# Sbte/RAILS

Hardware: AMD Instinct MI355X
Metric: RAILS iterations/sec (+ A*V SpMM HBM GB/s in roofline), m=1M rows/GPU, k=128, fp64 (higher is better)
Workload: dtype f64

## Files before the change

include/rails_hip.h:

```cpp
#ifndef RAILS_HIP_H
#define RAILS_HIP_H

#include <stddef.h>
#include <stdint.h>

#ifdef __cplusplus
extern "C" {
#endif

#define RAILS_OK 0
#define RAILS_EINVAL -1
#define RAILS_EHIP -2
#define RAILS_ENOMEM -3
#define RAILS_ELAPACK -4
#define RAILS_ECOMM -5
#define RAILS_ENODEV -6

typedef struct rails_ctx rails_ctx;
typedef struct rails_csr rails_csr;
typedef struct rails_panel rails_panel;

const char *rails_last_error(void);
const char *rails_version(void);

// ... 95 lines not shown

int rails_panel_gemm(rails_ctx *ctx, double alpha, const rails_panel *X, int xc0, int k, const double *C_host,
                     int ldc, int r, double beta, rails_panel *Y, int yc0);

int rails_ctx_enable_library_gemm(rails_ctx *ctx);
int rails_ctx_library_gemm_ready(const rails_ctx *ctx);

int rails_deferred_reserve(rails_ctx *ctx, int nslots, int64_t doubles_per_slot);
int rails_gram_deferred(rails_ctx *ctx, const rails_panel *X, int xc0, int a, const rails_panel *Y, int yc0, int b, int slot);
int rails_panel_gemm_deferred(rails_ctx *ctx, double alpha, const rails_panel *X, int xc0, int k, int slot, int ld, int r, double beta,
                              rails_panel *Y, int yc0);
int rails_chol_inverse_deferred(rails_ctx *ctx, int slot_in, int w, int slot_out);
int rails_update_gram_deferred(rails_ctx *ctx, double alpha, const rails_panel *X, int xc0, int k, const double *C_host, int ldc, int r,
                               rails_panel *Y, int yc0, int r2, int slot);
int rails_deferred_fetch(rails_ctx *ctx, int slot, int64_t n, double *host_out);

int rails_panel_gemm_wide(rails_ctx *ctx, double alpha, const rails_panel *X, int xc0, int k, const double *C_host, int ldc, int r,
                          double beta, rails_panel *Y, int yc0);

int rails_orthogonalize(rails_ctx *ctx, rails_panel *V, int k_old, int w, int method, int *used);
int rails_orthogonalize_deflated(rails_ctx *ctx, rails_panel *V, int k_old, int w, const rails_panel *N, int nc0, int q, int method, int *used);

int rails_resid_lanczos(rails_ctx *ctx, const rails_panel *AV, int avc0, const rails_panel *MV, int mvc0, int k,
                        const double *T_host, int ldt, const rails_panel *B, int bc0, int p, int L,
                        double *H_host, int ldh, int *steps);

int rails_lanczos_start(rails_ctx *ctx, const rails_panel *AV, int avc0, const rails_panel *MV, int mvc0, int k,
                        const rails_panel *B, int bc0, int p, double *sums_host);

int rails_lanczos_vectors(rails_ctx *ctx, const double *S_host, int lds, int w, rails_panel *Out, int oc0);
// ... 29 lines not shown
```

rails_amd/_lib.py:

```python
import ctypes as C
import os

_HERE = os.path.dirname(os.path.abspath(__file__))
LIB_PATH = os.path.join(_HERE, "lib", "librails_hip.so")

_dp = C.POINTER(C.c_double)
_ip = C.POINTER(C.c_int)
_i64p = C.POINTER(C.c_int64)
_i32p = C.POINTER(C.c_int32)
_vp = C.c_void_p

ALLREDUCE_FN = C.CFUNCTYPE(C.c_int, C.c_void_p, C.c_void_p, C.c_size_t, C.c_void_p)
HALO_FN = C.CFUNCTYPE(C.c_int, C.c_void_p, C.c_void_p, C.c_void_p, C.c_int, C.c_void_p)
APPLY_FN = C.CFUNCTYPE(C.c_int, C.c_void_p, C.c_int, C.c_void_p, C.c_int, C.c_int, C.c_void_p, C.c_int)

SIGNATURES = {
    "rails_last_error": (C.c_char_p, []),
    "rails_version": (C.c_char_p, []),
    "rails_ctx_create": (C.c_int, [C.c_int, _vp, C.POINTER(_vp)]),
    "rails_ctx_destroy": (C.c_int, [_vp]),
    "rails_ctx_sync": (C.c_int, [_vp]),
    "rails_ctx_stream": (_vp, [_vp]),
    "rails_ctx_set_meter": (C.c_int, [_vp, C.c_int]),
    "rails_ctx_enable_library_gemm": (C.c_int, [_vp]),
    "rails_ctx_library_gemm_ready": (C.c_int, [_vp]),
    "rails_deferred_reserve": (C.c_int, [_vp, C.c_int, C.c_int64]),
    "rails_gram_deferred": (C.c_int, [_vp, _vp, C.c_int, C.c_int, _vp, C.c_int, C.c_int, C.c_int]),
    "rails_update_gram_deferred": (C.c_int, [_vp, C.c_double, _vp, C.c_int, C.c_int, _dp, C.c_int, C.c_int, _vp, C.c_int, C.c_int, C.c_int]),
    "rails_panel_gemm_deferred": (C.c_int, [_vp, C.c_double, _vp, C.c_int, C.c_int, C.c_int, C.c_int, C.c_int, C.c_double, _vp, C.c_int]),
    "rails_chol_inverse_deferred": (C.c_int, [_vp, C.c_int, C.c_int, C.c_int]),
    "rails_deferred_fetch": (C.c_int, [_vp, C.c_int, C.c_int64, _dp]),
    "rails_ctx_stats": (C.c_int, [_vp, C.c_char_p, C.c_int]),
    "rails_ctx_set_seed": (C.c_int, [_vp, C.c_uint64, C.c_uint64]),
    "rails_ctx_rng_state": (C.c_int, [_vp, C.POINTER(C.c_uint64), C.POINTER(C.c_uint64)]),
    "rails_ctx_set_partition": (C.c_int, [_vp, C.c_int, C.c_int, C.c_int64, C.c_int64]),
    "rails_ctx_set_allreduce": (C.c_int, [_vp, ALLREDUCE_FN, _vp]),
    "rails_rccl_unique_id": (C.c_int, [_vp]),
    "rails_ctx_init_rccl": (C.c_int, [_vp, _vp, C.c_int, C.c_int]),
    "rails_ctx_set_rccl": (C.c_int, [_vp, _vp]),
    "rails_ctx_rccl_size": (C.c_int, [_vp]),
    "rails_csr_set_halo_counts": (C.c_int, [_vp, C.c_int, _i64p, _i64p]),
    "rails_csr_create": (C.c_int, [_vp, C.c_int64, C.c_int64, _i64p, _i32p, _dp, C.POINTER(_vp)]),
    "rails_csr_create_rect": (C.c_int, [_vp, C.c_int64, C.c_int64, _i64p, _i32p, _dp, C.POINTER(_vp)]),
    "rails_csr_create_callback": (C.c_int, [_vp, C.c_int64, APPLY_FN, _vp, C.POINTER(_vp)]),
    "rails_csr_destroy": (C.c_int, [_vp]),
    "rails_csr_rows": (C.c_int64, [_vp]),
# ... 103 lines not shown
```

rails_amd/csrc/ctx.hip:

```cpp
#include "rails_internal.h"

static thread_local char g_err[1024] = "";

void rails_set_error(const char *fmt, ...)
{
    va_list ap;
    va_start(ap, fmt);
    vsnprintf(g_err, sizeof(g_err), fmt, ap);
    va_end(ap);
}

extern "C" const char *rails_last_error(void) { return g_err; }
extern "C" const char *rails_version(void) { return "rails_amd 0.1 (gfx950)"; }


extern "C" int rails_ctx_create(int device, void *stream, rails_ctx **out)
{
    RAILS_REQUIRE(out != nullptr, "rails_ctx_create: out is null");
    int ndev = 0;
    hipError_t e = hipGetDeviceCount(&ndev);
    if (e != hipSuccess || ndev <= 0) {
        rails_set_error("rails_ctx_create: no HIP device visible (%s); the HIP path has no CPU fallback",
                        e == hipSuccess ? "device count 0" : hipGetErrorString(e));
        return RAILS_ENODEV;
// ... 39 lines not shown
extern "C" int rails_ctx_destroy(rails_ctx *c)
{
    if (!c) return RAILS_OK;
    hipSetDevice(c->device);
    rails_stream_sync(c);
    rails_lanczos_release(c);
    rails_rccl_release(c);
    rails_library_gemm_release(c);
    for (auto &fp : c->free_panels) hipFree(fp.second);
    c->free_panels.clear();
    if (c->ws) hipFree(c->ws);
    if (c->small) hipFree(c->small);
    if (c->pinned) hipHostFree(c->pinned);
    if (c->defer_dev) hipFree(c->defer_dev);
    if (c->defer_pin) hipHostFree(c->defer_pin);
    if (c->ev0) hipEventDestroy(c->ev0);
    if (c->ev1) hipEventDestroy(c->ev1);
    if (c->ev_h2d) hipEventDestroy(c->ev_h2d);
    for (hipEvent_t e : c->meter_events) hipEventDestroy(e);
    if (c->stream2) hipStreamDestroy(c->stream2);
    if (c->ev_fork) hipEventDestroy(c->ev_fork);
    if (c->ev_join) hipEventDestroy(c->ev_join);
    if (c->own_stream) hipStreamDestroy(c->stream);
    delete c;
    return RAILS_OK;
}

int rails_ctx_second_stream(rails_ctx *c)
{
    if (c->stream2) return RAILS_OK;
// ... 477 lines not shown
```

rails_amd/csrc/dense.hip:

```cpp
#include "rails_internal.h"

#include <dlfcn.h>
#include <atomic>
#include <mutex>

#include <algorithm>

namespace {

typedef double v4f64 __attribute__((ext_vector_type(4)));
typedef double v2f64 __attribute__((ext_vector_type(2)));

__device__ __forceinline__ v4f64 mfma_f64(double a, double b, v4f64 c)
{
    return __builtin_amdgcn_mfma_f64_16x16x4f64(a, b, c, 0, 0, 0);
}

struct OneSeg {
    const double *X;
    int ld;
    struct Row {
        const double *x;
    };
    __device__ int col(int c) const { return c; }
// ... 368 lines not shown
    RAILS_HIP_CHECK(hipMemcpyAsync(c->pinned, c->small, n * sizeof(double), hipMemcpyDeviceToHost, c->stream));
    RAILS_HIP_CHECK(rails_stream_sync(c));
    for (int j = 0; j < b; ++j) memcpy(C_host + (size_t)j * ldc, c->pinned + (size_t)j * a, sizeof(double) * a);
    return RAILS_OK;
}


namespace {

__global__ void k_compact_cols(const double *__restrict__ src, int ld, int k, int r, double *__restrict__ dst)
{
    const int64_t n = (int64_t)k * r;
    for (int64_t q = (int64_t)blockIdx.x * blockDim.x + threadIdx.x; q < n; q += (int64_t)gridDim.x * blockDim.x) dst[q] = src[(q / k) * ld + (q % k)];
}

__global__ __launch_bounds__(64) void k_small_chol(const double *__restrict__ G, int w, double *__restrict__ M)
{
    constexpr int LD = 49;
    __shared__ double S[48 * LD], Ri[48 * LD], d[48];
    const int t = threadIdx.x;
    const bool mine = t < w;
    for (int q = t; q < w * w; q += 64) S[(q / w) * LD + (q % w)] = G[q];
    __syncthreads();
    if (mine) d[t] = sqrt(S[t * LD + t]);
    __syncthreads();
    for (int q = t; q < w * w; q += 64) S[(q / w) * LD + (q % w)] /= d[q % w] * d[q / w];
    __syncthreads();
    for (int i = 0; i < w; ++i) {
        const double piv = sqrt(S[i * LD + i]);
        double rij = 0.0;
        if (mine && t >= i) rij = (t == i) ? piv : S[t * LD + i] / piv;
        __syncthreads();
        if (mine && t >= i) S[t * LD + i] = rij;
        __syncthreads();
        if (mine && t > i)
            for (int l = i + 1; l <= t; ++l) S[t * LD + l] -= S[l * LD + i] * rij;
        __syncthreads();
    }
    if (mine) {
        for (int l = 0; l < w; ++l) Ri[t * LD + l] = 0.0;
        for (int i = t; i >= 0; --i) {
            double s = (i == t) ? 1.0 : 0.0;
            for (int l = i + 1; l <= t; ++l) s -= S[l * LD + i] * Ri[t * LD + l];
            Ri[t * LD + i] = s / S[i * LD + i];
        }
    }
    __syncthreads();
    for (int q = t; q < w * w; q += 64) {
        const int j = q / w, i = q % w;
        M[q] = i <= j ? Ri[j * LD + i] / d[i] : 0.0;
    }
}

}

extern "C" int rails_deferred_reserve(rails_ctx *c, int nslots, int64_t doubles_per_slot)
{
    RAILS_REQUIRE(c && nslots >= 1 && doubles_per_slot >= 1, "rails_deferred_reserve: bad argument");
    hipSetDevice(c->device);
    if (c->defer_dev && c->defer_nslots >= nslots && c->defer_slot >= (size_t)doubles_per_slot) return RAILS_OK;
    RAILS_HIP_CHECK(rails_stream_sync(c));
    if (c->defer_dev) hipFree(c->defer_dev);
    if (c->defer_pin) hipHostFree(c->defer_pin);
    c->defer_dev = c->defer_pin = nullptr;
    const size_t slot = ((size_t)doubles_per_slot * 3 / 2 + 63) / 64 * 64, bytes = slot * (size_t)nslots * sizeof(double);
    c->n_dev_alloc++;
    RAILS_HIP_CHECK(hipMalloc((void **)&c->defer_dev, bytes));
    RAILS_HIP_CHECK(hipHostMalloc((void **)&c->defer_pin, bytes, hipHostMallocDefault));
    c->defer_slot = slot;
    c->defer_nslots = nslots;
    return RAILS_OK;
}

#define RAILS_SLOT_CHECK(slot, n, what)                                                                                                    \
    RAILS_REQUIRE(c && c->defer_dev && (slot) >= 0 && (slot) < c->defer_nslots && (size_t)(n) <= c->defer_slot,                            \
                  what ": slot %d / %lld doubles outside the arena (rails_deferred_reserve)", (int)(slot), (long long)(n))

extern "C" int rails_gram_deferred(rails_ctx *c, const rails_panel *X, int xc0, int a, const rails_panel *Y, int yc0, int b, int slot)
{
    if (c) hipSetDevice(c->device);
    RAILS_REQUIRE(c && X && Y, "rails_gram_deferred: null argument");
    RAILS_REQUIRE(a >= 1 && b >= 1 && xc0 >= 0 && yc0 >= 0 && xc0 + a <= X->cap && yc0 + b <= Y->cap && X->m == Y->m, "rails_gram_deferred: bad windows");
    const size_t n = (size_t)a * b;
// ... 210 lines not shown
}

extern "C" int rails_chol_inverse_deferred(rails_ctx *c, int slot_in, int w, int slot_out)
{
    if (c) hipSetDevice(c->device);
    RAILS_REQUIRE(c && w >= 1 && w <= 48 && slot_in != slot_out, "rails_chol_inverse_deferred: bad argument (w = %d)", w);
    RAILS_SLOT_CHECK(slot_in, (size_t)w * w, "rails_chol_inverse_deferred");
    RAILS_SLOT_CHECK(slot_out, (size_t)w * w, "rails_chol_inverse_deferred");
    RAILS_LAUNCH(k_small_chol, dim3(1), dim3(64), 0, c->stream, c->defer_dev + (size_t)slot_in * c->defer_slot, w, c->defer_dev + (size_t)slot_out * c->defer_slot);
    RAILS_HIP_CHECK(hipGetLastError());
    RAILS_HIP_CHECK(hipMemcpyAsync(c->defer_pin + (size_t)slot_out * c->defer_slot, c->defer_dev + (size_t)slot_out * c->defer_slot, (size_t)w * w * sizeof(double),
                                   hipMemcpyDeviceToHost, c->stream));
    return RAILS_OK;
}

extern "C" int rails_deferred_fetch(rails_ctx *c, int slot, int64_t n, double *host_out)
{
    RAILS_REQUIRE(host_out && n >= 0, "rails_deferred_fetch: bad argument");
    RAILS_SLOT_CHECK(slot, n, "rails_deferred_fetch");
    memcpy(host_out, c->defer_pin + (size_t)slot * c->defer_slot, (size_t)n * sizeof(double));
    return RAILS_OK;
}

int rails_panel_gemm_dev(rails_ctx *c, double alpha, const double *X, int ldx, int k, const double *C_dev, int r, double beta,
                         double *Y, int ldy, int64_t m)
{
    if (r <= 0 || m <= 0) return RAILS_OK;
    int vec_ok = ((((uintptr_t)X) & 15) == 0 && (ldx % 2) == 0) ? 1 : 0;
    int tr = (r + 15) / 16;
    if (tr <= 1)
        launch_pg<1, 32>(c, alpha, X, ldx, k, C_dev, r, beta, Y, ldy, m, vec_ok);
    else if (tr <= 2)
        launch_pg<2, 32>(c, alpha, X, ldx, k, C_dev, r, beta, Y, ldy, m, vec_ok);
    else if (tr <= 4)
// ... 184 lines not shown
```

rails_amd/csrc/dense_panel_gemm.inc:

```
    constexpr int RL = 16 * TR + 4;
    __shared__ double Cs[KC * RL];
    const int lane = threadIdx.x & 63;
    const int wave = threadIdx.x >> 6;
    const int li = lane & 15, kk = lane >> 4;
    const int64_t r0 = ((int64_t)blockIdx.x * 4 + wave) * 16;
    const int64_t myrow = r0 + li;
    const bool rowok = myrow < m;

    v4f64 acc[TR];
#pragma unroll
    for (int t = 0; t < TR; ++t) acc[t] = (v4f64){0.0, 0.0, 0.0, 0.0};

    const auto xrow = Xo.row(myrow);
    for (int kc = 0; kc < k; kc += KC) {
        __syncthreads();
        for (int idx = threadIdx.x; idx < KC * 16 * TR; idx += 256) {
            int kl = idx % KC, j = idx / KC;
            double v = 0.0;
            if (kc + kl < k && j < r) v = C[(kc + kl) + (int64_t)j * k];
            Cs[kl * RL + j] = v;
        }
        __syncthreads();
#pragma unroll
        for (int kb = 0; kb < KC; kb += 16) {
            const int kcol = kc + kb + 4 * kk;
            double xs[4];
            if (rowok && RAILS_PG_VEC4(kcol)) {
                const double *src = Xo.at(xrow, Xo.col(kcol));
                v2f64 t0 = *reinterpret_cast<const v2f64 *>(src);
                v2f64 t1 = *reinterpret_cast<const v2f64 *>(src + 2);
                xs[0] = t0.x;
                xs[1] = t0.y;
                xs[2] = t1.x;
                xs[3] = t1.y;
            } else {
#pragma unroll
                for (int s = 0; s < 4; ++s) xs[s] = (rowok && kcol + s < k) ? *Xo.at(xrow, Xo.col(kcol + s)) : 0.0;
            }
#pragma unroll
            for (int s = 0; s < 4; ++s) {
                const double *crow = &Cs[(kb + 4 * kk + s) * RL + li];
#pragma unroll
                for (int t = 0; t < TR; ++t) acc[t] = mfma_f64(xs[s], crow[16 * t], acc[t]);
            }
        }
    }
#pragma unroll
    for (int t = 0; t < TR; ++t) {
        const int j = 16 * t + li;
        if (j >= r) continue;
#pragma unroll
        for (int v = 0; v < 4; ++v) {
            const int64_t row = r0 + kk + 4 * v;
            if (row >= m) continue;
            double *dst = Yp + row * ldy + j;
            double val = alpha * acc[t][v];
            if (beta != 0.0) val += beta * (*dst);
            *dst = val;
        }
    }
#undef RAILS_PG_VEC4
```

rails_amd/csrc/rails_internal.h:

```cpp
#ifndef RAILS_INTERNAL_H
#define RAILS_INTERNAL_H

#include <hip/hip_runtime.h>

#include <cstdarg>
#include <cstdint>
#include <cstdio>
#include <cstring>
#include <ctime>
#include <string>
#include <vector>

#include "rails_hip.h"

void rails_set_error(const char *fmt, ...);

#define RAILS_HIP_CHECK(expr)                                                                      \
    do {                                                                                           \
        hipError_t e__ = (expr);                                                                   \
        if (e__ != hipSuccess) {                                                                   \
            rails_set_error("%s:%d: %s failed: %s", __FILE__, __LINE__, #expr, hipGetErrorString(e__)); \
            return RAILS_EHIP;                                                                     \
        }                                                                                          \
    } while (0)
// ... 32 lines not shown
    int rccl_nranks = 0, rccl_rank = 0;
    double *ws = nullptr;
    size_t ws_bytes = 0;
    std::vector<std::pair<size_t, double *>> free_panels;
    size_t free_panel_bytes = 0;
    double *small = nullptr;
    size_t small_bytes = 0;
    double *pinned = nullptr;
    size_t pinned_bytes = 0;
    hipEvent_t ev0 = nullptr, ev1 = nullptr;
    hipEvent_t ev_h2d = nullptr;
    bool h2d_pending = false;
    double *defer_dev = nullptr, *defer_pin = nullptr;
    size_t defer_slot = 0;
    int defer_nslots = 0;
    bool meter = false;
    std::vector<hipEvent_t> meter_events;
    int meter_open = 0;
    long meter_missed = 0;
    double gpu_busy_ms = 0.0;
    void *lz = nullptr;
    long n_orth_block = 0, n_orth_columnwise = 0, n_spmm_tiled = 0, n_spmm_planes = 0, n_spmm_overlapped = 0, n_spmm_sweep = 0, n_spmm_rowgather = 0, n_spmm_callback = 0, n_dev_alloc = 0, n_allreduce = 0, n_lanczos = 0, n_lanczos_start = 0, n_orth_repair = 0, n_update_gram_fused = 0, n_rowquad = 0;
};

constexpr int RAILS_METER_PAIRS = 512;
inline bool rails_meter_before(rails_ctx *c)
{
    if (!c->meter) return false;
    if (c->meter_open >= RAILS_METER_PAIRS) {
        c->meter_missed++;
// ... 151 lines not shown
```

rails_amd/csrc/solver_capi.cpp:

```cpp
#include <cmath>
#include <cstdio>
#include <cstring>
#include <map>
#include <string>
#include <vector>

#include <exception>
#include <new>

#include "rails/HipSolverOps.hpp"
#include "rails/SubspaceSolverOps.hpp"
#include "rails_solution.h"
#include "rails_solver.h"

void rails_set_error(const char *fmt, ...);

namespace
{

class ParameterList
{
    std::map<std::string, double> params_;

public:
// ... 226 lines not shown
    rails::SubspaceMultiVector Vc(basis, 1);
    if (s->have_V0) {
        Vc = rails::SubspaceMultiVector::Absorb(basis, s->V);
        Vc.set_orthogonalized(Vc.N());
    }
    int rc = solver.solve(Vc, s->T);
    s->null_rank = solver.nullspace_rank();
    if (rc == -2) return rc;
    s->V = Vc.materialise();
    s->V.set_orthogonalized(s->V.N());
    s->sub_trips = solver.trips();
    s->sub_hist = solver.residual_history();
    s->sub_profile = solver.profile();
    char buf[1536];
    snprintf(buf, sizeof(buf), "{\"dim\": %d, \"absorb\": %ld, \"absorb_columns\": %ld, \"one_by_one\": %ld, \"dropped\": %ld, \"compress\": %ld, \"materialise\": %ld, \"prefetched_random\": %ld, \"second_rounds\": %ld, \"delicate_blocks\": %ld, \"reprojected_blocks\": %ld, \"overlapped_blocks\": %ld, \"replaced_columns\": %ld, \"verified\": %d, \"verify_representation\": %.3e, \"verify_orthonormality\": %.3e, \"seconds\": {\"materialise\": %.4f, \"absorb\": %.4f, \"compress_qr\": %.4f, \"compress_rotate\": %.4f, "
             "\"compress_coefficients\": %.4f}}",
             basis->dim, basis->n_absorb, basis->n_absorb_cols, basis->n_single, basis->n_dropped, basis->n_compress, basis->n_materialise, basis->n_prefetched, basis->n_second_round, basis->n_delicate, basis->n_reprojected, basis->n_overlapped, basis->n_replaced, basis->verify ? 1 : 0, basis->verify_repr, basis->verify_orth,
             basis->t_materialise, basis->t_absorb, basis->t_qr, basis->t_rotate, basis->t_recoef);
    s->sub_stats = buf;
    if (basis->failed) {
        rails_set_error("coordinate-space back end: a device operation failed (%s)", rails_last_error());
        return -1000;
    }
    return rc;
}

extern "C" int rails_solver_solve(rails_solver *s, int *code, int *k)
{
    if (!s) return RAILS_EINVAL;
    const bool restart_from_solution = s->params.get("Restart from solution", 0.0) != 0.0;
    s->last_was_subspace = s->subspace && (s->have_V0 || !restart_from_solution);
    {
        rails::HipSolver::Projection proj;
// ... 149 lines not shown
```

rails_amd/include/rails/SubspaceWrappers.hpp:

```cpp
#ifndef RAILS_SUBSPACEWRAPPERS_HPP
#define RAILS_SUBSPACEWRAPPERS_HPP

#include <algorithm>
#include <atomic>
#include <chrono>
#include <cmath>
#include <cstdlib>
#include <cstring>
#include <iostream>
#include <memory>
#include <vector>

#include "rails/HipWrappers.hpp"

namespace rails
{

struct CoefStore {
    std::vector<double> c;
    int ld = 0, ncap = 0;
    bool in_basis = true;
    CoefStore(int ld_, int ncap_, bool in_basis_) : c((size_t)std::max(ld_, 1) * std::max(ncap_, 1), 0.0), ld(ld_), ncap(std::max(ncap_, 1)), in_basis(in_basis_) {}
    double *col(int j) { return c.data() + (size_t)j * ld; }
    const double *col(int j) const { return c.data() + (size_t)j * ld; }
};

class SubspaceBasis
{
public:
    rails_ctx *ctx;
    int64_t m_local, m_global;
    HipMultiVectorWrapper P, P2;
    int dim = 0;
    int row_cap;
    std::vector<std::weak_ptr<CoefStore>> live;
    long n_absorb = 0, n_absorb_cols = 0, n_single = 0, n_compress = 0, n_materialise = 0, n_dropped = 0, n_prefetched = 0, n_second_round = 0, n_delicate = 0, n_reprojected = 0;
    bool failed = false;
    long n_replaced = 0;
    double t_materialise = 0, t_absorb = 0, t_qr = 0, t_rotate = 0, t_recoef = 0;
    bool profile_sync = getenv("RAILS_SUBSPACE_PROFILE") != nullptr;
    bool trace = getenv("RAILS_SUBSPACE_TRACE") != nullptr;
    double reorth_survival = getenv("RAILS_SUBSPACE_REORTH") ? atof(getenv("RAILS_SUBSPACE_REORTH")) : 0.5;
    double slow_ms = getenv("RAILS_SUBSPACE_SLOW_MS") ? atof(getenv("RAILS_SUBSPACE_SLOW_MS")) : 0.0;
    struct Tick {
        SubspaceBasis *b;
        double *acc;
        const char *what;
        std::chrono::steady_clock::time_point t0;
        Tick(SubspaceBasis *bb, double *a, const char *w = "") : b(bb), acc(a), what(w)
        {
            if (b->profile_sync) rails_ctx_sync(b->ctx);
            t0 = std::chrono::steady_clock::now();
        }
        ~Tick()
        {
            if (b->profile_sync) rails_ctx_sync(b->ctx);
            const double dt = std::chrono::duration<double>(std::chrono::steady_clock::now() - t0).count();
            *acc += dt;
            if (b->slow_ms > 0.0 && dt * 1e3 > b->slow_ms)
                std::cerr << "[subspace] " << what << ": " << dt * 1e3 << " ms (dim " << b->dim << ", absorbs so far " << b->n_absorb << ")" << std::endl;
        }
    };
    std::shared_ptr<CoefStore> cached_random;
    bool cached_valid = false;
    bool prefetch_random = true;

    bool overlap = !(getenv("RAILS_SUBSPACE_OVERLAP") && atoi(getenv("RAILS_SUBSPACE_OVERLAP")) == 0);
    double overlap_min_survival = 1e-4;
    long n_overlapped = 0;
    struct Pending {
        bool active = false;
        int dim0 = 0, w = 0, w2 = 0;
        std::vector<double> Rfp;
        std::vector<double> g0diag;
    } pending;
    enum { SLOT_C2 = 0, SLOT_G = 1, SLOT_M1 = 2, SLOT_G2 = 3, SLOT_M2 = 4, N_SLOTS = 5 };

    SubspaceBasis(rails_ctx *c, int64_t ml, int64_t mg, int rows) : ctx(c), m_local(ml), m_global(mg), P(ml, std::max(rows, 16), c), row_cap(std::max(rows, 16))
    {
        P.set_global_rows(mg);
        P.resize(0);
    }
// ... 375 lines not shown
            d[j] = std::sqrt(Gp[j + (size_t)j * w]);
        }
        std::vector<double> R1((size_t)w * w);
        for (int b = 0; b < w; ++b)
            for (int a = 0; a < w; ++a) R1[a + (size_t)b * w] = Gp[a + (size_t)b * w] / (d[a] * d[b]);
        int info = 0;
        rails_dpotrf('U', w, R1.data(), w, &info);
        if (info != 0) return false;
        for (int a = 0; a < w; ++a)
            if (!(R1[a + (size_t)a * w] > 1e-2)) return false;
        if (!hip_ok(rails_deferred_reserve(ctx, N_SLOTS, (int64_t)(P.capacity() + 64) * (w <= 32 ? 32 : 48)), "rails_deferred_reserve")) return false;
        rails_panel *pp = P.panel();
        bool ok = true;
        if (w2 > 0) {
            ok = ok && hip_ok(rails_update_gram_deferred(ctx, -1.0, pp, 0, dim, CG.data(), dw, w, pp, dim, w2, SLOT_C2), "rails_update_gram_deferred");
            ok = ok && hip_ok(rails_panel_gemm_deferred(ctx, -1.0, pp, 0, dim, SLOT_C2, dim, w2, 1.0, pp, dim), "rails_panel_gemm_deferred");
        } else
            ok = ok && hip_ok(rails_panel_gemm(ctx, -1.0, pp, 0, dim, CG.data(), dw, w, 1.0, pp, dim), "rails_panel_gemm");
        ok = ok && hip_ok(rails_gram_deferred(ctx, pp, dim, w, pp, dim, w, SLOT_G), "rails_gram_deferred");
        ok = ok && hip_ok(rails_chol_inverse_deferred(ctx, SLOT_G, w, SLOT_M1), "rails_chol_inverse_deferred");
        ok = ok && hip_ok(rails_panel_gemm_deferred(ctx, 1.0, pp, dim, w, SLOT_M1, w, w, 0.0, pp, dim), "rails_panel_gemm_deferred");
        ok = ok && hip_ok(rails_gram_deferred(ctx, pp, dim, w, pp, dim, w, SLOT_G2), "rails_gram_deferred");
        ok = ok && hip_ok(rails_chol_inverse_deferred(ctx, SLOT_G2, w, SLOT_M2), "rails_chol_inverse_deferred");
        ok = ok && hip_ok(rails_panel_gemm_deferred(ctx, 1.0, pp, dim, w, SLOT_M2, w, w, 0.0, pp, dim), "rails_panel_gemm_deferred");
        if (!ok) return fail("the overlapped block orthogonalisation could not be queued");
        pending.active = true;
        pending.dim0 = dim;
        pending.w = w;
        pending.w2 = w2;
        pending.Rfp.assign((size_t)w * w, 0.0);
        pending.g0diag.resize(w);
        for (int b = 0; b < w; ++b) {
            pending.g0diag[b] = G0[b + (size_t)b * w];
            for (int a = 0; a <= b; ++a) {
                pending.Rfp[a + (size_t)b * w] = R1[a + (size_t)b * w] * d[b];
                coef[(dim + a) + (size_t)b * ld] = pending.Rfp[a + (size_t)b * w];
            }
        }
        if (w2 > 0) n_second_round++;
// ... 1 lines not shown
        static const long spoil = getenv("RAILS_SUBSPACE_TEST_SPOIL_PREDICTION") ? atol(getenv("RAILS_SUBSPACE_TEST_SPOIL_PREDICTION")) : 0;
        if (spoil > 0 && n_overlapped == spoil) {
            pending.Rfp[0] *= 1.01;
            coef[dim] = pending.Rfp[0];
        }
        dim += w;
        P.resize(dim);
        return true;
    }

    bool resolve_pending()
    {
        if (!pending.active) return !failed;
        pending.active = false;
        const int d0 = pending.dim0, w = pending.w, w2 = pending.w2;
        if (!hip_ok(rails_ctx_sync(ctx), "rails_ctx_sync")) return fail();
        std::vector<double> C2((size_t)d0 * w, 0.0), G((size_t)w * w), G2((size_t)w * w);
        bool ok = true;
        if (w2 > 0) ok = ok && hip_ok(rails_deferred_fetch(ctx, SLOT_C2, (int64_t)d0 * w2, C2.data()), "rails_deferred_fetch");
        ok = ok && hip_ok(rails_deferred_fetch(ctx, SLOT_G, (int64_t)w * w, G.data()), "rails_deferred_fetch");
        ok = ok && hip_ok(rails_deferred_fetch(ctx, SLOT_G2, (int64_t)w * w, G2.data()), "rails_deferred_fetch");
        if (!ok) return fail();
        auto factor = [&](std::vector<double> const &Gm, std::vector<double> &R, std::vector<double> &dd) {
            dd.resize(w);
            R.assign((size_t)w * w, 0.0);
            for (int j = 0; j < w; ++j) {
                if (!(Gm[j + (size_t)j * w] > 0.0) || !std::isfinite(Gm[j + (size_t)j * w])) return false;
                dd[j] = std::sqrt(Gm[j + (size_t)j * w]);
            }
            for (int b = 0; b < w; ++b)
                for (int a = 0; a < w; ++a) R[a + (size_t)b * w] = Gm[a + (size_t)b * w] / (dd[a] * dd[b]);
// ... 577 lines not shown
```

Baseline: 230.5.

## Fuse panel update with Gram accumulation and reduction with Cholesky inverse

In the overlapped block orthogonalisation, the correction GEMM now accumulates the Gram matrix of the updated block in the same pass through a new templated kernel. A single kernel reduces the per-block partials and computes the small Cholesky inverse, replacing separate gram, reduce and chol launches. This cuts passes over the tall panel and the number of kernel launches in the deferred chain. It adds a partials buffer, many template variants with register-pressure hints, and a separate code path enabled by default (switchable by an environment variable) that applies only when a second round runs.

```diff
diff --git a/include/rails_hip.h b/include/rails_hip.h
--- a/include/rails_hip.h
+++ b/include/rails_hip.h
@@ -133,6 +133,10 @@
 int rails_update_gram_deferred(rails_ctx *ctx, double alpha, const rails_panel *X, int xc0, int k, const double *C_host, int ldc, int r,
                                rails_panel *Y, int yc0, int r2, int slot);
 int rails_deferred_fetch(rails_ctx *ctx, int slot, int64_t n, double *host_out);
+int rails_panel_gemm_gram_deferred(rails_ctx *ctx, double alpha, const rails_panel *X, int xc0, int k, int slot, int ld, int r, rails_panel *Y,
+                                   int yc0, int rg, int slot_g);
+int rails_block_scale_gram_deferred(rails_ctx *ctx, rails_panel *Y, int yc0, int r, int slot_m, int slot_g);
+int rails_reduce_chol_inverse_deferred(rails_ctx *ctx, int slot_g, int w, int slot_m);
 
 int rails_panel_gemm_wide(rails_ctx *ctx, double alpha, const rails_panel *X, int xc0, int k, const double *C_host, int ldc, int r,
                           double beta, rails_panel *Y, int yc0);
diff --git a/rails_amd/_lib.py b/rails_amd/_lib.py
--- a/rails_amd/_lib.py
+++ b/rails_amd/_lib.py
@@ -30,6 +30,9 @@
     "rails_panel_gemm_deferred": (C.c_int, [_vp, C.c_double, _vp, C.c_int, C.c_int, C.c_int, C.c_int, C.c_int, C.c_double, _vp, C.c_int]),
     "rails_chol_inverse_deferred": (C.c_int, [_vp, C.c_int, C.c_int, C.c_int]),
     "rails_deferred_fetch": (C.c_int, [_vp, C.c_int, C.c_int64, _dp]),
+    "rails_panel_gemm_gram_deferred": (C.c_int, [_vp, C.c_double, _vp, C.c_int, C.c_int, C.c_int, C.c_int, C.c_int, _vp, C.c_int, C.c_int, C.c_int]),
+    "rails_block_scale_gram_deferred": (C.c_int, [_vp, _vp, C.c_int, C.c_int, C.c_int, C.c_int]),
+    "rails_reduce_chol_inverse_deferred": (C.c_int, [_vp, C.c_int, C.c_int, C.c_int]),
     "rails_ctx_stats": (C.c_int, [_vp, C.c_char_p, C.c_int]),
     "rails_ctx_set_seed": (C.c_int, [_vp, C.c_uint64, C.c_uint64]),
     "rails_ctx_rng_state": (C.c_int, [_vp, C.POINTER(C.c_uint64), C.POINTER(C.c_uint64)]),
diff --git a/rails_amd/csrc/ctx.hip b/rails_amd/csrc/ctx.hip
--- a/rails_amd/csrc/ctx.hip
+++ b/rails_amd/csrc/ctx.hip
@@ -77,6 +77,7 @@
     if (c->pinned) hipHostFree(c->pinned);
     if (c->defer_dev) hipFree(c->defer_dev);
     if (c->defer_pin) hipHostFree(c->defer_pin);
+    if (c->defer_part) hipFree(c->defer_part);
     if (c->ev0) hipEventDestroy(c->ev0);
     if (c->ev1) hipEventDestroy(c->ev1);
     if (c->ev_h2d) hipEventDestroy(c->ev_h2d);
diff --git a/rails_amd/csrc/dense.hip b/rails_amd/csrc/dense.hip
--- a/rails_amd/csrc/dense.hip
+++ b/rails_amd/csrc/dense.hip
@@ -406,17 +406,18 @@
     for (int64_t q = (int64_t)blockIdx.x * blockDim.x + threadIdx.x; q < n; q += (int64_t)gridDim.x * blockDim.x) dst[q] = src[(q / k) * ld + (q % k)];
 }
 
-__global__ __launch_bounds__(64) void k_small_chol(const double *__restrict__ G, int w, double *__restrict__ M)
+__device__ __forceinline__ void small_chol(const double *G, int w, double *__restrict__ M, double *__restrict__ Mmirror, int t, bool on)
 {
     constexpr int LD = 49;
     __shared__ double S[48 * LD], Ri[48 * LD], d[48];
-    const int t = threadIdx.x;
-    const bool mine = t < w;
-    for (int q = t; q < w * w; q += 64) S[(q / w) * LD + (q % w)] = G[q];
+    const bool mine = on && t < w;
+    if (on)
+        for (int q = t; q < w * w; q += 64) S[(q / w) * LD + (q % w)] = G[q];
     __syncthreads();
     if (mine) d[t] = sqrt(S[t * LD + t]);
     __syncthreads();
-    for (int q = t; q < w * w; q += 64) S[(q / w) * LD + (q % w)] /= d[q % w] * d[q / w];
+    if (on)
+        for (int q = t; q < w * w; q += 64) S[(q / w) * LD + (q % w)] /= d[q % w] * d[q / w];
     __syncthreads();
     for (int i = 0; i < w; ++i) {
         const double piv = sqrt(S[i * LD + i]);
@@ -438,11 +439,199 @@
         }
     }
     __syncthreads();
-    for (int q = t; q < w * w; q += 64) {
-        const int j = q / w, i = q % w;
-        M[q] = i <= j ? Ri[j * LD + i] / d[i] : 0.0;
-    }
-}
+    if (on)
+        for (int q = t; q < w * w; q += 64) {
+            const int j = q / w, i = q % w;
+            const double v = i <= j ? Ri[j * LD + i] / d[i] : 0.0;
+            M[q] = v;
+            if (Mmirror) Mmirror[q] = v;
+        }
+}
+
+__global__ __launch_bounds__(64) void k_small_chol(const double *__restrict__ G, int w, double *__restrict__ M) { small_chol(G, w, M, nullptr, threadIdx.x, true); }
+
+__global__ __launch_bounds__(1024) void k_reduce_chol(const double *__restrict__ partial, int64_t nslab, int w, double *__restrict__ G, double *__restrict__ Gmirror,
+                                                      double *__restrict__ M, double *__restrict__ Mmirror)
+{
+    __shared__ double sh[16][64];
+    __shared__ double Gs[48 * 48];
+    const int tx = threadIdx.x & 63, ty = threadIdx.x >> 6;
+    const int n = w * w, nu = w * (w + 1) / 2;
+    for (int u0 = 0; u0 < nu; u0 += 64) {
+        const int u = u0 + tx;
+        int j = 0;
+        while ((j + 1) * (j + 2) / 2 <= u) ++j;
+        const int i = u - j * (j + 1) / 2, e = i + j * w;
+        double s = 0.0;
+        if (u < nu)
+            for (int64_t t = ty; t < nslab; t += 16) s += partial[t * n + e];
+        sh[ty][tx] = s;
+        __syncthreads();
+        if (ty == 0 && u < nu) {
+            double r = 0.0;
+#pragma unroll
+            for (int g = 0; g < 16; ++g) r += sh[g][tx];
+            Gs[e] = r;
+            Gs[j + i * w] = r;
+        }
+        __syncthreads();
+    }
+    for (int q = threadIdx.x; q < n; q += 1024) {
+        G[q] = Gs[q];
+        Gmirror[q] = Gs[q];
+    }
+    small_chol(Gs, w, M, Mmirror, threadIdx.x, threadIdx.x < 64);
+}
+
+#ifndef RAILS_PGG_MINWAVES
+#define RAILS_PGG_MINWAVES 8
+#endif
+template <int TR, int KC, int NE, bool GRAM>
+__global__ __launch_bounds__(256) __attribute__((amdgpu_waves_per_eu(TR == 1 ? RAILS_PGG_MINWAVES : 1, 8))) void k_panel_gemm_gram(double alpha, const double *X, int ldx, int k, const double *__restrict__ C, int r, double beta, double *Yp,
+                                                          int ldy, int rg, int64_t m, int vec_ok, int64_t nbt, double *__restrict__ partial)
+{
+    const OneSeg Xo{X, ldx};
+    constexpr int NT = TR * (TR + 1) / 2;
+    const int wv = threadIdx.x >> 6, ln = threadIdx.x & 63, lkk = ln >> 4;
+    const int rgm = NE > 0 ? 16 * TR : rg;
+    v4f64 g[NT];
+    double ge[TR], gee = 0.0;
+#pragma unroll
+    for (int q = 0; q < NT; ++q) g[q] = (v4f64){0.0, 0.0, 0.0, 0.0};
+#pragma unroll
+    for (int t = 0; t < TR; ++t) ge[t] = 0.0;
+    for (int64_t bt = blockIdx.x; bt < nbt; bt += gridDim.x) {
+        double yn[TR][4], td[4], et = 0.0;
+#pragma unroll
+        for (int t = 0; t < TR; ++t)
+#pragma unroll
+            for (int v = 0; v < 4; ++v) yn[t][v] = 0.0;
+#pragma unroll
+        for (int v = 0; v < 4; ++v) td[v] = 0.0;
+#define RAILS_PG_WTILE (bt * 4 + wave)
+#define RAILS_PG_VEC4(c) (vec_ok && (c) + 4 <= k)
+#define RAILS_PG_STAGE(kc)                                                                                                                 \
+    if (NE == 2)                                                                                                                           \
+        for (int kl = threadIdx.x; kl < KC; kl += 256) Cs[kl * RL + 16 * TR] = (kc) + kl < k ? C[((kc) + kl) + (int64_t)(16 * TR) * k] : 0.0;   \
+    if (NE == 1 && GRAM && (kc) + KC >= k) {                                                                                               \
+        _Pragma("unroll") for (int v = 0; v < 4; ++v)                                                                                      \
+        {                                                                                                                                  \
+            const int64_t row = r0 + kk + 4 * v;                                                                                           \
+            const double t = Yp[(row < m ? row : m - 1) * ldy + 16 * TR];                                                                  \
+            td[v] = row < m ? t : 0.0;                                                                                                     \
+        }                                                                                                                                  \
+    }
+#define RAILS_PG_XS(x, crow)                                                                                                               \
+    if (NE == 2) et += (x) * (crow)[16 * TR - li];
+#define RAILS_PG_OUT(t, v, val) yn[t][v] = val;
+#include "dense_panel_gemm.inc"
+        if (NE == 2) {
+            double t = et;
+            t += __shfl_xor(t, 16, 64);
+            t += __shfl_xor(t, 32, 64);
+            const double tn = rowok ? alpha * t : 0.0;
+            if (rowok && kk == 0) Yp[myrow * ldy + 16 * TR] = tn;
+            if (GRAM) {
+#pragma unroll
+                for (int v = 0; v < 4; ++v) td[v] = __shfl(tn, kk + 4 * v, 64);
+            }
+        }
+        if (GRAM) {
+#pragma unroll
+            for (int t = 0; t < TR; ++t)
+#pragma unroll
+                for (int v = 0; v < 4; ++v) {
+                    const int j = 16 * t + li;
+                    const int64_t row = r0 + kk + 4 * v;
+                    if (j >= r && j < rgm && row < m) yn[t][v] = Yp[row * ldy + j];
+                }
+            int q = 0;
+#pragma unroll
+            for (int t = 0; t < TR; ++t)
+#pragma unroll
+                for (int t2 = t; t2 < TR; ++t2) {
+#pragma unroll
+                    for (int v = 0; v < 4; ++v) g[q] = mfma_f64(yn[t][v], yn[t2][v], g[q]);
+                    ++q;
+                }
+            if (NE > 0) {
+#pragma unroll
+                for (int v = 0; v < 4; ++v) {
+#pragma unroll
+                    for (int t = 0; t < TR; ++t) ge[t] += yn[t][v] * td[v];
+                    gee += td[v] * td[v];
+                }
+            }
+        }
+    }
+    if (GRAM) {
+        constexpr int PER = NT * 4 + (NE > 0 ? TR + 1 : 0);
+        __shared__ double red[PER * 64];
+        for (int w = 1; w < 4; ++w) {
+            if (wv == w) {
+#pragma unroll
+                for (int q = 0; q < NT; ++q)
+#pragma unroll
+                    for (int v = 0; v < 4; ++v) red[(q * 4 + v) * 64 + ln] = g[q][v];
+                if (NE > 0) {
+#pragma unroll
+                    for (int t = 0; t < TR; ++t) red[(NT * 4 + t) * 64 + ln] = ge[t];
+                    red[(NT * 4 + TR) * 64 + ln] = gee;
+                }
+            }
+            __syncthreads();
+            if (wv == 0) {
+#pragma unroll
+                for (int q = 0; q < NT; ++q)
+#pragma unroll
+                    for (int v = 0; v < 4; ++v) g[q][v] += red[(q * 4 + v) * 64 + ln];
+                if (NE > 0) {
+#pragma unroll
+                    for (int t = 0; t < TR; ++t) ge[t] += red[(NT * 4 + t) * 64 + ln];
+                    gee += red[(NT * 4 + TR) * 64 + ln];
+                }
+            }
+            __syncthreads();
+        }
+        if (wv == 0) {
+            const int li = ln & 15, kk = lkk;
+            double *P = partial + (int64_t)blockIdx.x * rg * rg;
+            int q = 0;
+#pragma unroll
+            for (int t = 0; t < TR; ++t)
+#pragma unroll
+                for (int t2 = t; t2 < TR; ++t2) {
+#pragma unroll
+                    for (int v = 0; v < 4; ++v) {
+                        const int ci = 16 * t + kk + 4 * v, cj = 16 * t2 + li;
+                        if (ci < rgm && cj < rgm && ci <= cj) {
+                            P[ci + (int64_t)cj * rg] = g[q][v];
+                            P[cj + (int64_t)ci * rg] = g[q][v];
+                        }
+                    }
+                    ++q;
+                }
+            if (NE > 0) {
+#pragma unroll
+                for (int t = 0; t < TR; ++t) {
+                    double s = ge[t];
+                    s += __shfl_xor(s, 16, 64);
+                    s += __shfl_xor(s, 32, 64);
+                    if (kk == 0) {
+                        P[(16 * t + li) + (int64_t)(16 * TR) * rg] = s;
+                        P[16 * TR + (int64_t)(16 * t + li) * rg] = s;
+                    }
+                }
+                double s = gee;
+                s += __shfl_xor(s, 16, 64);
+                s += __shfl_xor(s, 32, 64);
+                if (ln == 0) P[16 * TR + (int64_t)(16 * TR) * rg] = s;
+            }
+        }
+    }
+}
+
+constexpr int RAILS_TAIL_SLABS = 2048;
 
 }
 
@@ -455,10 +644,12 @@
     if (c->defer_dev) hipFree(c->defer_dev);
     if (c->defer_pin) hipHostFree(c->defer_pin);
     c->defer_dev = c->defer_pin = nullptr;
+    c->tail_slot = -1;
     const size_t slot = ((size_t)doubles_per_slot * 3 / 2 + 63) / 64 * 64, bytes = slot * (size_t)nslots * sizeof(double);
     c->n_dev_alloc++;
     RAILS_HIP_CHECK(hipMalloc((void **)&c->defer_dev, bytes));
     RAILS_HIP_CHECK(hipHostMalloc((void **)&c->defer_pin, bytes, hipHostMallocDefault));
+    RAILS_HIP_CHECK(hipHostGetDevicePointer((void **)&c->defer_pin_dev, c->defer_pin, 0));
     c->defer_slot = slot;
     c->defer_nslots = nslots;
     return RAILS_OK;
@@ -699,10 +890,138 @@
     return RAILS_OK;
 }
 
+namespace {
+
+int tail_part_reserve(rails_ctx *c, size_t bytes)
+{
+    if (c->defer_part && c->defer_part_bytes >= bytes) return RAILS_OK;
+    RAILS_HIP_CHECK(rails_stream_sync(c));
+    if (c->defer_part) RAILS_HIP_CHECK(hipFree(c->defer_part));
+    c->defer_part = nullptr;
+    c->defer_part_bytes = 0;
+    c->tail_slot = -1;
+    const size_t want = std::max(bytes, (size_t)RAILS_TAIL_SLABS * 33 * 33 * sizeof(double));
+    c->n_dev_alloc++;
+    RAILS_HIP_CHECK(hipMalloc((void **)&c->defer_part, want));
+    c->defer_part_bytes = want;
+    return RAILS_OK;
+}
+
+template <int TR, int NE>
+void launch_pgg(rails_ctx *c, bool gram, unsigned grid, double alpha, const double *X, int ldx, int k, const double *C, int r, double beta, double *Y, int ldy, int rg,
+                int64_t m, int vec_ok, int64_t nbt)
+{
+    if (gram)
+        RAILS_LAUNCH((k_panel_gemm_gram<TR, 32, NE, true>), dim3(grid), dim3(256), 0, c->stream, alpha, X, ldx, k, C, r, beta, Y, ldy, rg, m, vec_ok, nbt, c->defer_part);
+    else
+        RAILS_LAUNCH((k_panel_gemm_gram<TR, 32, NE, false>), dim3(grid), dim3(256), 0, c->stream, alpha, X, ldx, k, C, r, beta, Y, ldy, rg, m, vec_ok, nbt, c->defer_part);
+}
+
+int block_update_gram(rails_ctx *c, bool gram, bool own_tail, double alpha, const double *X, int ldx, int k, const double *C, int r, double beta, double *Y, int ldy,
+                      int rg, int64_t m, int64_t *nslab)
+{
+    const int vec_ok = ((((uintptr_t)X) & 15) == 0 && (ldx % 2) == 0) ? 1 : 0;
+    const int64_t nbt = (m + 63) / 64;
+    static const int per_cu = getenv("RAILS_TAIL_BLOCKS_PER_CU") ? atoi(getenv("RAILS_TAIL_BLOCKS_PER_CU")) : 8;
+    const unsigned grid = (unsigned)std::min<int64_t>(nbt, std::min<int64_t>(RAILS_TAIL_SLABS, per_cu * (int64_t)std::max(c->num_cu, 1)));
+    if (gram) RAILS_TRY(tail_part_reserve(c, (size_t)grid * rg * rg * sizeof(double)));
+    const bool tail = (rg == 17 || rg == 33) && (r < rg || (own_tail && beta == 0.0));
+    const int ne = !tail ? 0 : (r < rg ? 1 : 2);
+    const int tr = tail ? (rg - 1) / 16 : (rg + 15) / 16;
+#define RAILS_PGG_CASE(TR_, NE_)                                                                                                           \
+    if (tr == TR_ && ne == NE_) launch_pgg<TR_, NE_>(c, gram, grid, alpha, X, ldx, k, C, r, beta, Y, ldy, rg, m, vec_ok, nbt)
+    RAILS_PGG_CASE(1, 0);
+    RAILS_PGG_CASE(2, 0);
+    RAILS_PGG_CASE(3, 0);
+    RAILS_PGG_CASE(1, 1);
+    RAILS_PGG_CASE(2, 1);
+    RAILS_PGG_CASE(1, 2);
+    RAILS_PGG_CASE(2, 2);
+#undef RAILS_PGG_CASE
+    RAILS_HIP_CHECK(hipGetLastError());
+    *nslab = grid;
+    return RAILS_OK;
+}
+
+int block_gram_finish(rails_ctx *c, int slot, int w, int64_t nslab)
+{
+    const size_t n = (size_t)w * w;
+    double *out = c->defer_dev + (size_t)slot * c->defer_slot;
+    c->tail_slot = -1;
+    if (c->nranks <= 1 && !c->allreduce && !c->rccl && nslab > 0) {
+        c->tail_slot = slot;
+        c->tail_n = (int)n;
+        c->tail_nslab = nslab;
+        return RAILS_OK;
+    }
+    if (nslab > 0)
+        RAILS_LAUNCH(k_reduce_partials, dim3((unsigned)((n + 63) / 64)), dim3(1024), 0, c->stream, c->defer_part, nslab, (int64_t)n, out);
+    else
+        RAILS_HIP_CHECK(hipMemsetAsync(out, 0, n * sizeof(double), c->stream));
+    RAILS_HIP_CHECK(hipGetLastError());
+    RAILS_TRY(rails_allreduce_dev(c, out, n));
+    RAILS_HIP_CHECK(hipMemcpyAsync(c->defer_pin + (size_t)slot * c->defer_slot, out, n * sizeof(double), hipMemcpyDeviceToHost, c->stream));
+    return RAILS_OK;
+}
+
+}
+
+extern "C" int rails_panel_gemm_gram_deferred(rails_ctx *c, double alpha, const rails_panel *X, int xc0, int k, int slot, int ld, int r, rails_panel *Y, int yc0,
+                                              int rg, int slot_g)
+{
+    if (c) hipSetDevice(c->device);
+    RAILS_REQUIRE(c && X && Y, "rails_panel_gemm_gram_deferred: null argument");
+    RAILS_REQUIRE(k >= 1 && r >= 1 && rg >= r && rg <= 48 && ld >= k && xc0 >= 0 && yc0 >= 0 && xc0 + k <= X->cap && yc0 + rg <= Y->cap && X->m == Y->m && slot != slot_g,
+                  "rails_panel_gemm_gram_deferred: bad shapes");
+    RAILS_SLOT_CHECK(slot, (size_t)ld * r, "rails_panel_gemm_gram_deferred");
+    RAILS_SLOT_CHECK(slot_g, (size_t)rg * rg, "rails_panel_gemm_gram_deferred");
+    if (X->d == Y->d) RAILS_REQUIRE(xc0 + k <= yc0 || yc0 + rg <= xc0, "rails_panel_gemm_gram_deferred: overlapping windows of one panel");
+    int64_t nslab = 0;
+    if (X->m > 0) {
+        const double *C = c->defer_dev + (size_t)slot * c->defer_slot;
+        if (ld != k) {
+            RAILS_TRY(rails_small_reserve(c, (size_t)k * r * sizeof(double)));
+            RAILS_LAUNCH(k_compact_cols, dim3((unsigned)std::min<int64_t>(256, ((int64_t)k * r + 255) / 256)), dim3(256), 0, c->stream, C, ld, k, r, c->small);
+            C = c->small;
+        }
+        RAILS_TRY(block_update_gram(c, true, false, alpha, X->d + xc0, X->ld, k, C, r, 1.0, Y->d + yc0, Y->ld, rg, X->m, &nslab));
+    }
+    return block_gram_finish(c, slot_g, rg, nslab);
+}
+
+extern "C" int rails_block_scale_gram_deferred(rails_ctx *c, rails_panel *Y, int yc0, int r, int slot_m, int slot_g)
+{
+    if (c) hipSetDevice(c->device);
+    RAILS_REQUIRE(c && Y, "rails_block_scale_gram_deferred: null argument");
+    RAILS_REQUIRE(r >= 1 && r <= 48 && yc0 >= 0 && yc0 + r <= Y->cap && slot_m != slot_g, "rails_block_scale_gram_deferred: bad shapes");
+    RAILS_SLOT_CHECK(slot_m, (size_t)r * r, "rails_block_scale_gram_deferred");
+    if (slot_g >= 0) RAILS_SLOT_CHECK(slot_g, (size_t)r * r, "rails_block_scale_gram_deferred");
+    int64_t nslab = 0;
+    if (Y->m > 0)
+        RAILS_TRY(block_update_gram(c, slot_g >= 0, true, 1.0, Y->d + yc0, Y->ld, r, c->defer_dev + (size_t)slot_m * c->defer_slot, r, 0.0, Y->d + yc0, Y->ld, r, Y->m, &nslab));
+    return slot_g >= 0 ? block_gram_finish(c, slot_g, r, nslab) : RAILS_OK;
+}
+
+extern "C" int rails_reduce_chol_inverse_deferred(rails_ctx *c, int slot_g, int w, int slot_m)
+{
+    if (c) hipSetDevice(c->device);
+    RAILS_REQUIRE(c && w >= 1 && w <= 48 && slot_g != slot_m, "rails_reduce_chol_inverse_deferred: bad argument (w = %d)", w);
+    RAILS_SLOT_CHECK(slot_g, (size_t)w * w, "rails_reduce_chol_inverse_deferred");
+    RAILS_SLOT_CHECK(slot_m, (size_t)w * w, "rails_reduce_chol_inverse_deferred");
+    if (c->tail_slot != slot_g) return rails_chol_inverse_deferred(c, slot_g, w, slot_m);
+    RAILS_REQUIRE(c->tail_n == w * w, "rails_reduce_chol_inverse_deferred: the partials waiting for slot %d are not %d x %d", slot_g, w, w);
+    c->tail_slot = -1;
+    const size_t og = (size_t)slot_g * c->defer_slot, om = (size_t)slot_m * c->defer_slot;
+    RAILS_LAUNCH(k_reduce_chol, dim3(1), dim3(1024), 0, c->stream, c->defer_part, c->tail_nslab, w, c->defer_dev + og, c->defer_pin_dev + og, c->defer_dev + om, c->defer_pin_dev + om);
+    RAILS_HIP_CHECK(hipGetLastError());
+    return RAILS_OK;
+}
+
 extern "C" int rails_deferred_fetch(rails_ctx *c, int slot, int64_t n, double *host_out)
 {
     RAILS_REQUIRE(host_out && n >= 0, "rails_deferred_fetch: bad argument");
     RAILS_SLOT_CHECK(slot, n, "rails_deferred_fetch");
+    RAILS_REQUIRE(slot != c->tail_slot, "rails_deferred_fetch: slot %d waits for rails_reduce_chol_inverse_deferred", slot);
     memcpy(host_out, c->defer_pin + (size_t)slot * c->defer_slot, (size_t)n * sizeof(double));
     return RAILS_OK;
 }
diff --git a/rails_amd/csrc/dense_panel_gemm.inc b/rails_amd/csrc/dense_panel_gemm.inc
--- a/rails_amd/csrc/dense_panel_gemm.inc
+++ b/rails_amd/csrc/dense_panel_gemm.inc
@@ -1,9 +1,15 @@
+#ifndef RAILS_PG_WTILE
+#define RAILS_PG_WTILE ((int64_t)blockIdx.x * 4 + wave)
+#define RAILS_PG_STAGE(kc)
+#define RAILS_PG_XS(x, crow)
+#define RAILS_PG_OUT(t, v, val)
+#endif
     constexpr int RL = 16 * TR + 4;
     __shared__ double Cs[KC * RL];
     const int lane = threadIdx.x & 63;
     const int wave = threadIdx.x >> 6;
     const int li = lane & 15, kk = lane >> 4;
-    const int64_t r0 = ((int64_t)blockIdx.x * 4 + wave) * 16;
+    const int64_t r0 = RAILS_PG_WTILE * 16;
     const int64_t myrow = r0 + li;
     const bool rowok = myrow < m;
 
@@ -20,6 +26,7 @@
             if (kc + kl < k && j < r) v = C[(kc + kl) + (int64_t)j * k];
             Cs[kl * RL + j] = v;
         }
+        RAILS_PG_STAGE(kc)
         __syncthreads();
 #pragma unroll
         for (int kb = 0; kb < KC; kb += 16) {
@@ -42,6 +49,7 @@
                 const double *crow = &Cs[(kb + 4 * kk + s) * RL + li];
 #pragma unroll
                 for (int t = 0; t < TR; ++t) acc[t] = mfma_f64(xs[s], crow[16 * t], acc[t]);
+                RAILS_PG_XS(xs[s], crow)
             }
         }
     }
@@ -57,6 +65,11 @@
             double val = alpha * acc[t][v];
             if (beta != 0.0) val += beta * (*dst);
             *dst = val;
+            RAILS_PG_OUT(t, v, val)
         }
     }
 #undef RAILS_PG_VEC4
+#undef RAILS_PG_WTILE
+#undef RAILS_PG_STAGE
+#undef RAILS_PG_XS
+#undef RAILS_PG_OUT
diff --git a/rails_amd/csrc/rails_internal.h b/rails_amd/csrc/rails_internal.h
--- a/rails_amd/csrc/rails_internal.h
+++ b/rails_amd/csrc/rails_internal.h
@@ -70,6 +70,10 @@
     double *defer_dev = nullptr, *defer_pin = nullptr;
     size_t defer_slot = 0;
     int defer_nslots = 0;
+    double *defer_part = nullptr, *defer_pin_dev = nullptr;
+    size_t defer_part_bytes = 0;
+    int tail_slot = -1, tail_n = 0;
+    int64_t tail_nslab = 0;
     bool meter = false;
     std::vector<hipEvent_t> meter_events;
     int meter_open = 0;
diff --git a/rails_amd/csrc/solver_capi.cpp b/rails_amd/csrc/solver_capi.cpp
--- a/rails_amd/csrc/solver_capi.cpp
+++ b/rails_amd/csrc/solver_capi.cpp
@@ -264,9 +264,9 @@
     s->sub_profile = solver.profile();
     char buf[1536];
     snprintf(buf, sizeof(buf), "{\"dim\": %d, \"absorb\": %ld, \"absorb_columns\": %ld, \"one_by_one\": %ld, \"dropped\": %ld, \"compress\": %ld, \"materialise\": %ld, \"prefetched_random\": %ld, \"second_rounds\": %ld, \"delicate_blocks\": %ld, \"reprojected_blocks\": %ld, \"overlapped_blocks\": %ld, \"replaced_columns\": %ld, \"verified\": %d, \"verify_representation\": %.3e, \"verify_orthonormality\": %.3e, \"seconds\": {\"materialise\": %.4f, \"absorb\": %.4f, \"compress_qr\": %.4f, \"compress_rotate\": %.4f, "
-             "\"compress_coefficients\": %.4f}}",
+             "\"compress_coefficients\": %.4f, \"overlap_wait\": %.6f}, \"fused_tail\": %d}",
              basis->dim, basis->n_absorb, basis->n_absorb_cols, basis->n_single, basis->n_dropped, basis->n_compress, basis->n_materialise, basis->n_prefetched, basis->n_second_round, basis->n_delicate, basis->n_reprojected, basis->n_overlapped, basis->n_replaced, basis->verify ? 1 : 0, basis->verify_repr, basis->verify_orth,
-             basis->t_materialise, basis->t_absorb, basis->t_qr, basis->t_rotate, basis->t_recoef);
+             basis->t_materialise, basis->t_absorb, basis->t_qr, basis->t_rotate, basis->t_recoef, basis->t_wait, basis->fused_tail ? 1 : 0);
     s->sub_stats = buf;
     if (basis->failed) {
         rails_set_error("coordinate-space back end: a device operation failed (%s)", rails_last_error());
diff --git a/rails_amd/include/rails/SubspaceWrappers.hpp b/rails_amd/include/rails/SubspaceWrappers.hpp
--- a/rails_amd/include/rails/SubspaceWrappers.hpp
+++ b/rails_amd/include/rails/SubspaceWrappers.hpp
@@ -38,6 +38,7 @@
     bool failed = false;
     long n_replaced = 0;
     double t_materialise = 0, t_absorb = 0, t_qr = 0, t_rotate = 0, t_recoef = 0;
+    double t_wait = 0;
     bool profile_sync = getenv("RAILS_SUBSPACE_PROFILE") != nullptr;
     bool trace = getenv("RAILS_SUBSPACE_TRACE") != nullptr;
     double reorth_survival = getenv("RAILS_SUBSPACE_REORTH") ? atof(getenv("RAILS_SUBSPACE_REORTH")) : 0.5;
@@ -66,6 +67,7 @@
     bool prefetch_random = true;
 
     bool overlap = !(getenv("RAILS_SUBSPACE_OVERLAP") && atoi(getenv("RAILS_SUBSPACE_OVERLAP")) == 0);
+    bool fused_tail = !(getenv("RAILS_SUBSPACE_FUSED_TAIL") && atoi(getenv("RAILS_SUBSPACE_FUSED_TAIL")) == 0);
     double overlap_min_survival = 1e-4;
     long n_overlapped = 0;
     struct Pending {
@@ -471,15 +473,23 @@
         bool ok = true;
         if (w2 > 0) {
             ok = ok && hip_ok(rails_update_gram_deferred(ctx, -1.0, pp, 0, dim, CG.data(), dw, w, pp, dim, w2, SLOT_C2), "rails_update_gram_deferred");
-            ok = ok && hip_ok(rails_panel_gemm_deferred(ctx, -1.0, pp, 0, dim, SLOT_C2, dim, w2, 1.0, pp, dim), "rails_panel_gemm_deferred");
+            if (!fused_tail) ok = ok && hip_ok(rails_panel_gemm_deferred(ctx, -1.0, pp, 0, dim, SLOT_C2, dim, w2, 1.0, pp, dim), "rails_panel_gemm_deferred");
         } else
             ok = ok && hip_ok(rails_panel_gemm(ctx, -1.0, pp, 0, dim, CG.data(), dw, w, 1.0, pp, dim), "rails_panel_gemm");
-        ok = ok && hip_ok(rails_gram_deferred(ctx, pp, dim, w, pp, dim, w, SLOT_G), "rails_gram_deferred");
-        ok = ok && hip_ok(rails_chol_inverse_deferred(ctx, SLOT_G, w, SLOT_M1), "rails_chol_inverse_deferred");
-        ok = ok && hip_ok(rails_panel_gemm_deferred(ctx, 1.0, pp, dim, w, SLOT_M1, w, w, 0.0, pp, dim), "rails_panel_gemm_deferred");
-        ok = ok && hip_ok(rails_gram_deferred(ctx, pp, dim, w, pp, dim, w, SLOT_G2), "rails_gram_deferred");
-        ok = ok && hip_ok(rails_chol_inverse_deferred(ctx, SLOT_G2, w, SLOT_M2), "rails_chol_inverse_deferred");
-        ok = ok && hip_ok(rails_panel_gemm_deferred(ctx, 1.0, pp, dim, w, SLOT_M2, w, w, 0.0, pp, dim), "rails_panel_gemm_deferred");
+        if (w2 > 0 && fused_tail) {
+            ok = ok && hip_ok(rails_panel_gemm_gram_deferred(ctx, -1.0, pp, 0, dim, SLOT_C2, dim, w2, pp, dim, w, SLOT_G), "rails_panel_gemm_gram_deferred");
+            ok = ok && hip_ok(rails_reduce_chol_inverse_deferred(ctx, SLOT_G, w, SLOT_M1), "rails_reduce_chol_inverse_deferred");
+            ok = ok && hip_ok(rails_block_scale_gram_deferred(ctx, pp, dim, w, SLOT_M1, SLOT_G2), "rails_block_scale_gram_deferred");
+            ok = ok && hip_ok(rails_reduce_chol_inverse_deferred(ctx, SLOT_G2, w, SLOT_M2), "rails_reduce_chol_inverse_deferred");
+            ok = ok && hip_ok(rails_block_scale_gram_deferred(ctx, pp, dim, w, SLOT_M2, -1), "rails_block_scale_gram_deferred");
+        } else {
+            ok = ok && hip_ok(rails_gram_deferred(ctx, pp, dim, w, pp, dim, w, SLOT_G), "rails_gram_deferred");
+            ok = ok && hip_ok(rails_chol_inverse_deferred(ctx, SLOT_G, w, SLOT_M1), "rails_chol_inverse_deferred");
+            ok = ok && hip_ok(rails_panel_gemm_deferred(ctx, 1.0, pp, dim, w, SLOT_M1, w, w, 0.0, pp, dim), "rails_panel_gemm_deferred");
+            ok = ok && hip_ok(rails_gram_deferred(ctx, pp, dim, w, pp, dim, w, SLOT_G2), "rails_gram_deferred");
+            ok = ok && hip_ok(rails_chol_inverse_deferred(ctx, SLOT_G2, w, SLOT_M2), "rails_chol_inverse_deferred");
+            ok = ok && hip_ok(rails_panel_gemm_deferred(ctx, 1.0, pp, dim, w, SLOT_M2, w, w, 0.0, pp, dim), "rails_panel_gemm_deferred");
+        }
         if (!ok) return fail("the overlapped block orthogonalisation could not be queued");
         pending.active = true;
         pending.dim0 = dim;
@@ -511,7 +521,10 @@
         if (!pending.active) return !failed;
         pending.active = false;
         const int d0 = pending.dim0, w = pending.w, w2 = pending.w2;
-        if (!hip_ok(rails_ctx_sync(ctx), "rails_ctx_sync")) return fail();
+        {
+            Tick tick(this, &t_wait, "resolve: wait for the deferred chain");
+            if (!hip_ok(rails_ctx_sync(ctx), "rails_ctx_sync")) return fail();
+        }
         std::vector<double> C2((size_t)d0 * w, 0.0), G((size_t)w * w), G2((size_t)w * w);
         bool ok = true;
         if (w2 > 0) ok = ok && hip_ok(rails_deferred_fetch(ctx, SLOT_C2, (int64_t)d0 * w2, C2.data()), "rails_deferred_fetch");
```

Result: slower. 225.0 (-2.4%).
